# ykojima4020/mae_clip

Hardware: NVIDIA B200
Metric: contrastive loss fwd+bwd samples/s (higher is better)
Workload: dtype fp32 (fp16 hi+lo split operands, 3 tcgen05 passes, fp32 accumulate)

## Files before the change

mae_clip_b200/csrc/clip_loss_tc.cu:

```cuda
#include <stdlib.h>
#include <string.h>

#include "clip_loss.cuh"
#include "tc_ptx.cuh"

#include <type_traits>

namespace mc {
namespace tc {

using namespace ptx;


constexpr int kTileN = 128;
constexpr int kRowsCta = 64;
constexpr int kChunkBytes = 64 * 128;
constexpr int kThreads = 384;
constexpr int kEpiThreads = 256;
constexpr int kMaxSplit = 16;
constexpr int kIssuers = 1;

enum Phase { kStats = 0, kRowLoss = 1, kBwd = 2, kStatsZ = 3, kBwdW = 4, kBwdP = 5 };

constexpr int kOffA = 0;
// ... 1123 lines not shown
  __syncthreads();
  if (threadIdx.x < 32) {
    double t = (threadIdx.x < (blockDim.x >> 5)) ? sm[threadIdx.x] : 0.0;
    t = warp_sum(t);
    if (threadIdx.x == 0) *out = (float)t;
  }
}

__global__ void __launch_bounds__(1024) wscale_kernel(const float* __restrict__ r, const float* __restrict__ c,
                                                      const float* __restrict__ rz, const float* __restrict__ q, int B,
                                                      const float* __restrict__ scale,
                                                      const float* __restrict__ norm_i,
                                                      const float* __restrict__ norm_t, float inv_tau, float tau,
                                                      float* __restrict__ out) {
  __shared__ float sm[10][32];
  float v[10] = {-INFINITY, -INFINITY, 0.f, 0.f, 0.f, 0.f, -INFINITY, -INFINITY, -INFINITY, -INFINITY};
  auto take = [&](float ri, float ci, float zi, float qi, float ni, float nt) {
    v[0] = fmaxf(v[0], ri); v[1] = fmaxf(v[1], ci); v[2] = fmaxf(v[2], qi);
    v[4] = fmaxf(v[4], ni); v[5] = fmaxf(v[5], nt);
    v[6] = fmaxf(v[6], zi); v[7] = fmaxf(v[7], -ri); v[8] = fmaxf(v[8], -ci); v[9] = fmaxf(v[9], -zi);
  };
  int i0 = 0;
  const uintptr_t align = reinterpret_cast<uintptr_t>(r) | reinterpret_cast<uintptr_t>(c) | reinterpret_cast<uintptr_t>(rz) |
                          reinterpret_cast<uintptr_t>(q) | reinterpret_cast<uintptr_t>(norm_i) |
                          reinterpret_cast<uintptr_t>(norm_t);
  if ((align & 15) == 0) {
    const int B4 = B >> 2;
    for (int i = threadIdx.x; i < B4; i += blockDim.x) {
      const float4 a = reinterpret_cast<const float4*>(r)[i], b4 = reinterpret_cast<const float4*>(c)[i];
      const float4 z = reinterpret_cast<const float4*>(rz)[i], qq = reinterpret_cast<const float4*>(q)[i];
      const float4 ni = reinterpret_cast<const float4*>(norm_i)[i], nt = reinterpret_cast<const float4*>(norm_t)[i];
      take(a.x, b4.x, z.x, qq.x, ni.x, nt.x);
      take(a.y, b4.y, z.y, qq.y, ni.y, nt.y);
      take(a.z, b4.z, z.z, qq.z, ni.z, nt.z);
      take(a.w, b4.w, z.w, qq.w, ni.w, nt.w);
    }
    i0 = B4 << 2;
  }
  for (int i = i0 + threadIdx.x; i < B; i += blockDim.x) take(r[i], c[i], rz[i], q[i], norm_i[i], norm_t[i]);
  for (int k = 0; k < 10; ++k) {
    v[k] = warp_max(v[k]);
    if ((threadIdx.x & 31) == 0) sm[k][threadIdx.x >> 5] = v[k];
  }
  __syncthreads();
  if (threadIdx.x < 32) {
    for (int k = 0; k < 10; ++k) v[k] = warp_max(sm[k][threadIdx.x]);
    if (threadIdx.x == 0) {
      v[3] = scale[1];
      const float gmax = fmaxf(v[0] + v[1] + 2.f * v[4] * v[5] * inv_tau, 1.f);
      const float b1 = (2.f + v[2]) * v[3] * inv_tau;
      const float b3 = 2.f * gmax * v[3] * 0.5f * tau;
      const float bound = fmaxf(fmaxf(b1, b3), 1e-30f);
      int e;
      frexpf(bound, &e);
      int k = 15 - e;
      k = k < -60 ? -60 : (k > 60 ? 60 : k);
      out[0] = ldexpf(1.f, k);
      const float kL2e = 1.4426950408889634f;
      const float hi_rc = fmaxf(v[0], v[1]), lo_rc = -fmaxf(v[7], v[8]);
      const float hi_z = v[6], lo_z = -v[9];
      const bool fast = (hi_rc - lo_rc) * kL2e <= 60.f && (hi_z - lo_z) * kL2e <= 60.f;
      out[1] = fast ? 1.f : 0.f;
      out[2] = 0.5f * (hi_rc + lo_rc) * kL2e;
      out[3] = 0.5f * (hi_z + lo_z) * kL2e;
    }
  }
}

__global__ void __launch_bounds__(256) bwd_finalize_kernel(const float* __restrict__ part, int nsplit, int bpad,
                                                           int b, int D, float inv_2B,
                                                           const float* __restrict__ grad_loss,
                                                           const float* __restrict__ wscale,
                                                           float* __restrict__ dT, float* __restrict__ dI,
                                                           const int* __restrict__ gate = nullptr, int gate_want = 0) {
  if (gate != nullptr && *gate != gate_want) return;
  const float scale = (grad_loss ? *grad_loss : 1.f) * inv_2B / *wscale;
  const size_t n4 = (size_t)b * D / 4;
  const size_t plane = (size_t)bpad * D;
  for (size_t i = (size_t)blockIdx.x * blockDim.x + threadIdx.x; i < n4; i += (size_t)gridDim.x * blockDim.x) {
    float4 at = make_float4(0.f, 0.f, 0.f, 0.f), ai = at;
    for (int s = 0; s < nsplit; ++s) {
      const float4 a = reinterpret_cast<const float4*>(part + (size_t)s * 2 * plane)[i];
      const float4 c = reinterpret_cast<const float4*>(part + ((size_t)s * 2 + 1) * plane)[i];
      at.x += a.x; at.y += a.y; at.z += a.z; at.w += a.w;
      ai.x += c.x; ai.y += c.y; ai.z += c.z; ai.w += c.w;
    }
    reinterpret_cast<float4*>(dT)[i] = make_float4(at.x * scale, at.y * scale, at.z * scale, at.w * scale);
    reinterpret_cast<float4*>(dI)[i] = make_float4(ai.x * scale, ai.y * scale, ai.z * scale, ai.w * scale);
  }
}

constexpr int kCgThreads = 256;
constexpr int kCgStageA = 2 * 8192;
constexpr int kCgStages = 6;
constexpr int kCgMaxSplit = 8;
struct ColGradParams {
  int Bp, D;
  int w_rows;
  int row_offset;
  int j_first;
  int n_jblocks;
  int j_end;
  int ksplit, steps_per_split, steps;
  float* part;
  const int* gate;
};
__device__ __forceinline__ uint64_t smem_desc_mn_sw128(uint32_t saddr, uint32_t lbo_bytes) {
  uint64_t d = 0;
  d |= static_cast<uint64_t>((saddr & 0x3FFFFu) >> 4);
  d |= static_cast<uint64_t>(lbo_bytes >> 4) << 16;
  d |= static_cast<uint64_t>(1024 >> 4) << 32;
  d |= static_cast<uint64_t>(1) << 46;
  d |= static_cast<uint64_t>(2) << 61;
  return d;
}
__global__ void __launch_bounds__(kCgThreads, 1)
colgrad_kernel(const __grid_constant__ CUtensorMap map_w, const __grid_constant__ CUtensorMap map_t,
               const ColGradParams p) {
  if (p.gate != nullptr && *p.gate != 1) return;
  extern __shared__ uint8_t smem_raw[];
  const uint32_t raw = smem_u32(smem_raw);
  const uint32_t base = (raw + 1023u) & ~1023u;
  uint8_t* const sbase = smem_raw + (base - raw);
  const int D = p.D;
  const uint32_t b_bytes = (uint32_t)(D / 2) * 128u;
  const uint32_t stage_bytes = kCgStageA + b_bytes;
  const uint32_t bar0 = base + kCgStages * stage_bytes;
  auto bar = [&](int i) -> uint32_t { return bar0 + 8u * i; };
  enum { kFull = 0, kEmpty = kCgStages, kAccFull = 2 * kCgStages, kAccEmpty = 2 * kCgStages + 2, kBars = 2 * kCgStages + 4 };
  uint32_t* const tmem_slot = reinterpret_cast<uint32_t*>(sbase + kCgStages * stage_bytes + 8 * kBars);

  const int warp = __shfl_sync(0xffffffffu, (int)(threadIdx.x >> 5), 0), lane = threadIdx.x & 31;
  const uint32_t rank = cluster_ctarank();
  const bool leader = rank == 0;
  const int pair_id = blockIdx.x >> 1, npairs = gridDim.x >> 1;
  const int njobs = p.n_jblocks * p.ksplit;

  if (threadIdx.x == 0) {
    for (int s = 0; s < kCgStages; ++s) { mbar_init(bar(kFull + s), 1); mbar_init(bar(kEmpty + s), 1); }
    for (int i = 0; i < 2; ++i) { mbar_init(bar(kAccFull + i), 1); mbar_init(bar(kAccEmpty + i), 2 * 128); }
    fence_mbar_init();
    prefetch_tmap(&map_w);
    prefetch_tmap(&map_t);
  }
  if (warp == 1) {
    tmem_alloc_pair(smem_u32(tmem_slot), 512);
    tmem_relinquish_pair();
  }
  tc_fence_before();
  cluster_sync_all();
  tc_fence_after();
  const uint32_t tmem_base = *tmem_slot;

  if (warp == 0) {
    if (elect_one()) {
      uint32_t it = 0;
      for (int job = pair_id; job < njobs; job += npairs) {
        const int jb = job / p.ksplit, ks = job % p.ksplit;
        const int j0 = p.j_first + jb * 256 + (int)rank * 128;
        const int s0 = ks * p.steps_per_split, s1 = min(s0 + p.steps_per_split, p.steps);
        for (int st = s0; st < s1; ++st, ++it) {
          const uint32_t slot = it % kCgStages, par = (it / kCgStages) & 1;
          mbar_wait(bar(kEmpty + slot), par ^ 1);
          const uint32_t fb = bar(kFull + slot), sa = base + slot * stage_bytes;
          if (leader) mbar_arrive_expect_tx(fb, 2u * stage_bytes);
          const int i0 = st * 64;
          tma_load_2d_pair(sa, &map_w, fb, j0, i0);
          tma_load_2d_pair(sa + 8192, &map_w, fb, j0 + 64, i0);
          tma_load_2d_pair(sa + kCgStageA, &map_t, fb, p.row_offset + i0, D + (int)rank * (D / 2));
        }
      }
    }
  } else if (warp == 1) {
    if (leader && elect_one()) {
      const uint32_t idesc = idesc_f16(256, D) | (1u << 15);
      uint32_t it = 0, jj = 0;
      for (int job = pair_id; job < njobs; job += npairs) {
        const int ks = job % p.ksplit;
        const int s0 = ks * p.steps_per_split, s1 = min(s0 + p.steps_per_split, p.steps);
        if (s0 >= s1) continue;
        const uint32_t buf = jj & 1, use = jj >> 1;
        ++jj;
        mbar_wait(bar(kAccEmpty + buf), (use & 1) ^ 1);
        tc_fence_after();
        const uint32_t tacc = tmem_base + buf * (uint32_t)D;
        for (int st = s0; st < s1; ++st, ++it) {
          const uint32_t slot = it % kCgStages, par = (it / kCgStages) & 1;
          mbar_wait(bar(kFull + slot), par);
          tc_fence_after();
          const uint32_t sa = base + slot * stage_bytes;
          const uint64_t bd = smem_desc_sw128(sa + kCgStageA);
#pragma unroll
          for (int k4 = 0; k4 < 4; ++k4)
            mma_f16_pair(tacc, smem_desc_mn_sw128(sa + k4 * 2048, 8192), desc_advance_k(bd, k4), idesc,
                         (st > s0 || k4 > 0) ? 1u : 0u);
          mma_commit_pair(bar(kEmpty + slot), 3);
        }
        mma_commit_pair(bar(kAccFull + buf), 3);
      }
    }
  } else if (warp >= 4) {
    const int q = warp - 4;
    uint32_t jj = 0;
    for (int job = pair_id; job < njobs; job += npairs) {
      const int jb = job / p.ksplit, ks = job % p.ksplit;
      const int lrow = jb * 256 + (int)rank * 128 + q * 32 + lane;
      const bool ok = p.j_first + lrow < p.j_end;
      const int s0 = ks * p.steps_per_split;
      const bool empty = s0 >= p.steps;
      const uint32_t buf = jj & 1, use = jj >> 1;
      if (!empty) ++jj;
      float* out = p.part + ((size_t)ks * p.n_jblocks * 256 + lrow) * D;
      if (!empty) {
        mbar_wait(bar(kAccFull + buf), use & 1);
        tc_fence_after();
      }
      for (int c0 = 0; c0 < D; c0 += 32) {
        float v[32];
        if (!empty) {
          tmem_ld32(tmem_base + ((uint32_t)(q * 32) << 16) + buf * (uint32_t)D + c0, v);
          tmem_ld_wait();
        } else {
#pragma unroll
          for (int e = 0; e < 32; ++e) v[e] = 0.f;
        }
        if (ok) {
#pragma unroll
          for (int e = 0; e < 32; e += 4)
            *reinterpret_cast<float4*>(out + c0 + e) = make_float4(v[e], v[e + 1], v[e + 2], v[e + 3]);
        }
      }
      if (!empty) {
        tc_fence_before();
        mbar_arrive_cluster(bar(kAccEmpty + buf), 0);
      }
    }
  }
  tc_fence_before();
  cluster_sync_all();
  if (warp == 1) tmem_dealloc_pair(tmem_base, 512);
}

__global__ void __launch_bounds__(256) bwd_rows_finalize_kernel(const float* __restrict__ part, int nsplit, int bpad,
                                                                int b, int D, float inv_2B,
                                                                const float* __restrict__ grad_loss,
                                                                const float* __restrict__ wscale,
                                                                float* __restrict__ dT, float* __restrict__ dIz) {
  const float scale = (grad_loss ? *grad_loss : 1.f) * inv_2B / *wscale;
  const size_t n4 = (size_t)b * D / 4;
  const size_t plane = (size_t)bpad * D;
  for (size_t i = (size_t)blockIdx.x * blockDim.x + threadIdx.x; i < n4; i += (size_t)gridDim.x * blockDim.x) {
    float4 at = make_float4(0.f, 0.f, 0.f, 0.f), ai = at;
    for (int s = 0; s < nsplit; ++s) {
      const float4 a = reinterpret_cast<const float4*>(part + (size_t)s * 2 * plane)[i];
      const float4 c = reinterpret_cast<const float4*>(part + ((size_t)s * 2 + 1) * plane)[i];
      at.x += a.x; at.y += a.y; at.z += a.z; at.w += a.w;
      ai.x += c.x; ai.y += c.y; ai.z += c.z; ai.w += c.w;
    }
    reinterpret_cast<float4*>(dT)[i] = make_float4(at.x * scale, at.y * scale, at.z * scale, at.w * scale);
    reinterpret_cast<float4*>(dIz)[i] = ai;
  }
}
__global__ void __launch_bounds__(256) bwd_rows_split_finalize_kernel(const float* __restrict__ part_r, int nsplit_r,
                                                                      size_t plane_r, const float* __restrict__ part_p,
                                                                      size_t plane_p, int b, int D, float inv_2B,
                                                                      const float* __restrict__ grad_loss,
                                                                      const float* __restrict__ wscale,
                                                                      float* __restrict__ dT, float* __restrict__ dIz,
                                                                      const int* __restrict__ gate) {
  if (gate != nullptr && *gate != 1) return;
  const float scale = (grad_loss ? *grad_loss : 1.f) * inv_2B / *wscale;
  const size_t n4 = (size_t)b * D / 4;
  for (size_t i = (size_t)blockIdx.x * blockDim.x + threadIdx.x; i < n4; i += (size_t)gridDim.x * blockDim.x) {
    float4 at = reinterpret_cast<const float4*>(part_p)[i];
    for (int s = 0; s < nsplit_r; ++s) {
      const float4 a = reinterpret_cast<const float4*>(part_r + (size_t)s * plane_r)[i];
      at.x += a.x; at.y += a.y; at.z += a.z; at.w += a.w;
    }
    reinterpret_cast<float4*>(dT)[i] = make_float4(at.x * scale, at.y * scale, at.z * scale, at.w * scale);
    reinterpret_cast<float4*>(dIz)[i] = reinterpret_cast<const float4*>(part_p + plane_p)[i];
  }
}
__global__ void __launch_bounds__(256) bwd_cols_finalize_kernel(const float* __restrict__ part, int ksplit, size_t plane,
                                                                int rows, int D, float inv_2B,
                                                                const float* __restrict__ grad_loss,
                                                                const float* __restrict__ wscale,
                                                                const float* __restrict__ dIz, float* __restrict__ dI,
                                                                const int* __restrict__ gate) {
  if (gate != nullptr && *gate != 1) return;
  const float scale = (grad_loss ? *grad_loss : 1.f) * inv_2B / *wscale;
  const size_t n4 = (size_t)rows * D / 4;
  for (size_t i = (size_t)blockIdx.x * blockDim.x + threadIdx.x; i < n4; i += (size_t)gridDim.x * blockDim.x) {
    float4 a = dIz ? reinterpret_cast<const float4*>(dIz)[i] : make_float4(0.f, 0.f, 0.f, 0.f);
    for (int s = 0; s < ksplit; ++s) {
      const float4 c = reinterpret_cast<const float4*>(part + (size_t)s * plane)[i];
      a.x += c.x; a.y += c.y; a.z += c.z; a.w += c.w;
    }
    reinterpret_cast<float4*>(dI)[i] = make_float4(a.x * scale, a.y * scale, a.z * scale, a.w * scale);
  }
}

constexpr int kRgThreads = 384;
constexpr int kRgRowsCta = 128;
constexpr int kRgSlotBytes = 32768;
constexpr int kRgSlots = 3;
constexpr int kRgOffA = 0;
constexpr int kRgOffRing = 65536;
constexpr int kRgOffW = kRgOffRing + kRgSlots * kRgSlotBytes;
constexpr int kRgOffXT = kRgOffW + 2 * 16384;
constexpr int kRgOffConst = kRgOffXT + 2 * 16384;
constexpr int kRgOffBar = kRgOffConst + 2048;
constexpr int kRgSmemBytes = kRgOffBar + 256 + 512;
enum RgBar {
  kRgFull0 = 0, kRgEmpty0 = 3, kRgAFull = 6, kRgJobDone = 7, kRgTmemFull0 = 8, kRgTmemEmpty0 = 10, kRgWFull0 = 12,
  kRgXTFull0 = 14, kRgGradDone0 = 16, kRgAccFull = 18, kRgAccEmpty = 19, kRgCstFull0 = 20, kRgCstEmpty0 = 22, kRgNumBars = 24
};
struct RowGradParams {
  int b, B, Bp, D, row_offset;
  int n_row_blocks, n_tiles, nsplit, tiles_per_split, bpad;
  float inv_tau;
  const float* scale;
  const float *r, *c, *q;
  const float* wscale;
  float* part;
  __half* wout;
  const int* gate;
};
template <int PASSES>
__global__ void __launch_bounds__(kRgThreads, 1)
rowgrad_kernel(const __grid_constant__ CUtensorMap map_a_hi, const __grid_constant__ CUtensorMap map_a_lo,
               const __grid_constant__ CUtensorMap map_b_hi, const __grid_constant__ CUtensorMap map_b_lo,
               const __grid_constant__ CUtensorMap map_t, const RowGradParams p) {
  if (p.gate != nullptr && *p.gate != 1) return;
  extern __shared__ __align__(1024) uint8_t smem_raw[];
  const uint32_t raw = smem_u32(smem_raw);
  const uint32_t base = (raw + 1023u) & ~1023u;
  if (base - raw > 512u) __trap();
  uint8_t* const sbase = smem_raw + (base - raw);
  const uint32_t bar0 = base + kRgOffBar;
  auto bar = [&](int i) -> uint32_t { return bar0 + 8u * i; };
  uint32_t* const tmem_slot = reinterpret_cast<uint32_t*>(sbase + kRgOffBar + 8 * kRgNumBars);

  const int warp = __shfl_sync(0xffffffffu, (int)(threadIdx.x >> 5), 0), lane = threadIdx.x & 31;
  const uint32_t rank = cluster_ctarank();
  const bool leader = rank == 0;
  const int pair_id = blockIdx.x >> 1, npairs = gridDim.x >> 1;
  const int D = p.D, nkc = D >> 6;
  const int njobs = p.n_row_blocks * p.nsplit;
  const uint32_t xt_bytes = (uint32_t)(D / 2) * 128u;

  if (threadIdx.x == 0) {
    for (int s = 0; s < kRgSlots; ++s) { mbar_init(bar(kRgFull0 + s), 1); mbar_init(bar(kRgEmpty0 + s), 1); }
    mbar_init(bar(kRgAFull), 1);
    mbar_init(bar(kRgJobDone), 1);
    for (int i = 0; i < 2; ++i) {
      mbar_init(bar(kRgTmemFull0 + i), 1);
      mbar_init(bar(kRgTmemEmpty0 + i), 2 * 256);
      mbar_init(bar(kRgWFull0 + i), 2 * 128);
      mbar_init(bar(kRgXTFull0 + i), 1);
      mbar_init(bar(kRgGradDone0 + i), 1);
      mbar_init(bar(kRgCstFull0 + i), 32);
      mbar_init(bar(kRgCstEmpty0 + i), 256);
    }
    mbar_init(bar(kRgAccFull), 1);
    mbar_init(bar(kRgAccEmpty), 2 * 256);
    fence_mbar_init();
    prefetch_tmap(&map_a_hi); prefetch_tmap(&map_a_lo); prefetch_tmap(&map_b_hi); prefetch_tmap(&map_b_lo);
    prefetch_tmap(&map_t);
  }
  if (warp == 1) {
    tmem_alloc_pair(smem_u32(tmem_slot), 512);
    tmem_relinquish_pair();
  }
  tc_fence_before();
  cluster_sync_all();
  tc_fence_after();
  const uint32_t tmem_base = *tmem_slot;
  constexpr uint32_t kAcc = 256;

  if (warp == 0) {
    if (elect_one()) {
      uint32_t it = 0, jj = 0;
      for (int job = pair_id; job < njobs; job += npairs, ++jj) {
        const int rb = job / p.nsplit, sp = job % p.nsplit;
        const int row_a = p.row_offset + rb * 256 + (int)rank * kRgRowsCta;
        const int t0 = sp * p.tiles_per_split, t1 = min(t0 + p.tiles_per_split, p.n_tiles);
        mbar_wait(bar(kRgJobDone), (jj & 1) ^ 1);
        if (leader) mbar_arrive_expect_tx(bar(kRgAFull), 2u * (uint32_t)nkc * 16384u);
        for (int c = 0; c < nkc; ++c) tma_load_2d_pair(base + kRgOffA + c * 16384, &map_a_hi, bar(kRgAFull), D + c * 64, row_a);
        for (int t = t0; t < t1; ++t) {
          const int j0 = t * kTileN + 64 * (int)rank;
          for (int c = 0; c < nkc; ++c, ++it) {
            const uint32_t slot = it % kRgSlots, par = (it / kRgSlots) & 1;
            mbar_wait(bar(kRgEmpty0 + slot), par ^ 1);
            const uint32_t fb = bar(kRgFull0 + slot), sb = base + kRgOffRing + slot * kRgSlotBytes;
            if (leader) mbar_arrive_expect_tx(fb, PASSES == 3 ? 2u * kRgSlotBytes : 2u * 8192u);
            if (PASSES == 3) tma_load_2d_pair(sb, &map_a_lo, fb, D + c * 64, row_a);
            tma_load_2d_pair(sb + 16384, &map_b_hi, fb, c * 64, j0);
            if (PASSES == 3) tma_load_2d_pair(sb + 24576, &map_b_lo, fb, c * 64, j0);
          }
        }
      }
    }
  } else if (warp == 2) {
    if (elect_one()) {
      uint32_t tt = 0;
      for (int job = pair_id; job < njobs; job += npairs) {
        const int sp = job % p.nsplit;
        const int t0 = sp * p.tiles_per_split, t1 = min(t0 + p.tiles_per_split, p.n_tiles);
        for (int t = t0; t < t1; ++t, ++tt) {
          for (int h = 0; h < 2; ++h) {
            mbar_wait(bar(kRgGradDone0 + h), (tt & 1) ^ 1);
            const uint32_t fb = bar(kRgXTFull0 + h);
            if (leader) mbar_arrive_expect_tx(fb, 2u * xt_bytes);
            tma_load_2d_pair(base + kRgOffXT + h * 16384, &map_t, fb, t * kTileN + 64 * h, (int)rank * (D / 2));
          }
        }
      }
    }
  } else if (warp == 3) {
    float* const consts = reinterpret_cast<float*>(sbase + kRgOffConst);
    const float kL2e = 1.4426950408889634f;
    const bool fast = p.wscale[1] != 0.f;
    const float m_rc = p.wscale[2];
    uint32_t tt = 0;
    for (int job = pair_id; job < njobs; job += npairs) {
      const int sp = job % p.nsplit;
      const int t0 = sp * p.tiles_per_split, t1 = min(t0 + p.tiles_per_split, p.n_tiles);
      for (int t = t0; t < t1; ++t, ++tt) {
        float vc[4], vq[4];
#pragma unroll
        for (int u = 0; u < 4; ++u) {
          const int jcol = t * kTileN + lane + 32 * u;
          const bool ok = jcol < p.B;
          vc[u] = ok ? p.c[jcol] : 0.f;
          vq[u] = ok ? p.q[jcol] : 0.f;
        }
        mbar_wait(bar(kRgCstEmpty0 + (tt & 1)), ((tt >> 1) & 1) ^ 1);
        float* dst = consts + (tt & 1) * 256;
#pragma unroll
        for (int u = 0; u < 4; ++u) {
          const int col = lane + 32 * u;
          const bool ok = t * kTileN + col < p.B;
          const float c2 = vc[u] * kL2e;
          if (fast) {
            dst[col] = ok ? ex2f(m_rc - c2) * vq[u] : 0.f;
          } else {
            dst[col] = -c2;
            dst[128 + col] = vq[u];
          }
        }
        mbar_arrive_local(bar(kRgCstFull0 + (tt & 1)));
      }
    }
  } else if (warp == 1) {
    if (leader && elect_one()) {
      constexpr uint32_t idesc_s = idesc_f16(256, kTileN);
      const uint32_t idesc_g = idesc_f16(256, D);
      const uint32_t tDT = tmem_base + kAcc;
      uint32_t it = 0, tt = 0, gt = 0, jj = 0;
      auto grad_tile = [&](bool first_of_job) {
        for (int h = 0; h < 2; ++h) {
          mbar_wait(bar(kRgWFull0 + h), gt & 1);
          mbar_wait(bar(kRgXTFull0 + h), gt & 1);
          tc_fence_after();
          const uint64_t wd = smem_desc_sw128(base + kRgOffW + h * 16384), xd = smem_desc_sw128(base + kRgOffXT + h * 16384);
#pragma unroll
          for (int ks = 0; ks < 4; ++ks)
            mma_f16_pair(tDT, desc_advance_k(wd, ks), desc_advance_k(xd, ks), idesc_g, (first_of_job && h == 0 && ks == 0) ? 0u : 1u);
          mma_commit_pair(bar(kRgGradDone0 + h), 3);
        }
        ++gt;
      };
      for (int job = pair_id; job < njobs; job += npairs, ++jj) {
        const int sp = job % p.nsplit;
        const int t0 = sp * p.tiles_per_split, t1 = min(t0 + p.tiles_per_split, p.n_tiles);
        mbar_wait(bar(kRgAFull), jj & 1);
        tc_fence_after();
        for (int t = t0; t < t1; ++t, ++tt) {
          const uint32_t buf = tt & 1, use = tt >> 1;
          mbar_wait(bar(kRgTmemEmpty0 + buf), (use & 1) ^ 1);
          tc_fence_after();
          const uint32_t tS = tmem_base + buf * 128;
          for (int c = 0; c < nkc; ++c, ++it) {
            const uint32_t slot = it % kRgSlots, par = (it / kRgSlots) & 1;
            mbar_wait(bar(kRgFull0 + slot), par);
            tc_fence_after();
            const uint32_t sb = base + kRgOffRing + slot * kRgSlotBytes;
            const uint64_t aT = smem_desc_sw128(base + kRgOffA + c * 16384), aTl = smem_desc_sw128(sb);
            const uint64_t bI = smem_desc_sw128(sb + 16384), bIl = smem_desc_sw128(sb + 24576);
#pragma unroll
            for (int ks = 0; ks < 4; ++ks) {
              const uint64_t kT = desc_advance_k(aT, ks), kb = desc_advance_k(bI, ks);
              mma_f16_pair(tS, kT, kb, idesc_s, (c > 0 || ks > 0) ? 1u : 0u);
              if (PASSES == 3) {
                mma_f16_pair(tS, kT, desc_advance_k(bIl, ks), idesc_s, 1u);
                mma_f16_pair(tS, desc_advance_k(aTl, ks), kb, idesc_s, 1u);
              }
            }
            mma_commit_pair(bar(kRgEmpty0 + slot), 3);
          }
          mma_commit_pair(bar(kRgTmemFull0 + buf), 3);
          if (t == t0) {
            mbar_wait(bar(kRgAccEmpty), (jj & 1) ^ 1);
            tc_fence_after();
          } else {
            grad_tile(t - 1 == t0);
          }
        }
        grad_tile(t1 - 1 == t0);
        mma_commit_pair(bar(kRgAccFull), 3);
        mma_commit_pair(bar(kRgJobDone), 3);
      }
    }
    __syncwarp();
  } else if (warp >= 4) {
    const int q4 = warp & 3, h = (warp - 4) >> 2;
    const int m = q4 * 32 + lane;
    const uint32_t lane_field = (uint32_t)(q4 * 32) << 16;
    const float* const consts = reinterpret_cast<const float*>(sbase + kRgOffConst);
    const float kL2e = 1.4426950408889634f;
    const float inv_s = p.scale[1], inv_s2 = p.scale[2];
    const float cS2 = inv_s2 * p.inv_tau * kL2e;
    const float wS = inv_s * p.inv_tau * p.wscale[0];
    const bool fast = p.wscale[1] != 0.f;
    const float m_rc = p.wscale[2];
    uint32_t tt = 0, jj = 0;
    for (int job = pair_id; job < njobs; job += npairs, ++jj) {
      const int rb = job / p.nsplit, sp = job % p.nsplit;
      const int t0 = sp * p.tiles_per_split, t1 = min(t0 + p.tiles_per_split, p.n_tiles);
      const int lrow = rb * 256 + (int)rank * kRgRowsCta + m;
      const int gi = p.row_offset + lrow;
      const bool row_ok = lrow < p.b;
      const float r2_i = row_ok ? p.r[gi] * kL2e : 0.f;
      const float fC_i = ex2f(r2_i - m_rc);
      const float wrow = row_ok ? wS : 0.f;
      for (int t = t0; t < t1; ++t, ++tt) {
        const uint32_t buf = tt & 1, use = tt >> 1;
        mbar_wait(bar(kRgCstFull0 + (tt & 1)), (tt >> 1) & 1);
        const float* cst = consts + (tt & 1) * 256 + 64 * h;
        mbar_wait(bar(kRgTmemFull0 + buf), use & 1);
        tc_fence_after();
        const uint32_t tS = tmem_base + buf * 128 + lane_field + 64 * h;
        uint32_t wp[32];
#pragma unroll
        for (int half = 0; half < 2; ++half) {
          float v[32];
          tmem_ld32(tS + 32 * half, v);
          tmem_ld_wait();
          if (half == 1) {
            tc_fence_before();
            mbar_arrive_cluster(bar(kRgTmemEmpty0 + buf), 0);
          }
#pragma unroll
          for (int e = 0; e < 32; e += 4) {
            const float4 f0 = *reinterpret_cast<const float4*>(cst + 32 * half + e);
            const float4 f1 = fast ? make_float4(0.f, 0.f, 0.f, 0.f) : *reinterpret_cast<const float4*>(cst + 128 + 32 * half + e);
            const float k0[4] = {f0.x, f0.y, f0.z, f0.w}, k1[4] = {f1.x, f1.y, f1.z, f1.w};
            float w[4];
#pragma unroll
            for (int u = 0; u < 4; ++u) {
              const float a = v[e + u];
              const float e1 = ex2f(fmaf(a, cS2, -r2_i));
              float dS;
              if (fast) dS = e1 * fmaf(fC_i, k0[u], 1.f);
              else dS = fmaf(ex2f(fmaf(a, cS2, k0[u])), k1[u], e1);
              w[u] = dS * wrow;
            }
            __half2 x = __floats2half2_rn(w[0], w[1]), y = __floats2half2_rn(w[2], w[3]);
            wp[16 * half + (e >> 1)] = *reinterpret_cast<uint32_t*>(&x);
            wp[16 * half + (e >> 1) + 1] = *reinterpret_cast<uint32_t*>(&y);
          }
        }
        mbar_wait(bar(kRgGradDone0 + h), (tt & 1) ^ 1);
        uint8_t* wsm = sbase + kRgOffW + h * 16384 + m * 128;
#pragma unroll
        for (int k = 0; k < 8; ++k)
          *reinterpret_cast<uint4*>(wsm + ((k ^ (m & 7)) * 16)) = make_uint4(wp[4 * k], wp[4 * k + 1], wp[4 * k + 2], wp[4 * k + 3]);
        fence_proxy_async_smem();
        mbar_arrive_cluster(bar(kRgWFull0 + h), 0);
        uint4* wg = reinterpret_cast<uint4*>(p.wout + (size_t)lrow * p.Bp + (size_t)t * kTileN + 64 * h);
#pragma unroll
        for (int k = 0; k < 8; ++k) wg[k] = make_uint4(wp[4 * k], wp[4 * k + 1], wp[4 * k + 2], wp[4 * k + 3]);
        mbar_arrive_local(bar(kRgCstEmpty0 + (tt & 1)));
      }
      mbar_wait(bar(kRgAccFull), jj & 1);
      tc_fence_after();
      float* out = p.part + ((size_t)sp * p.bpad + lrow) * D + h * (D / 2);
      for (int c0 = 0; c0 < D / 2; c0 += 32) {
        float v[32];
        tmem_ld32(tmem_base + lane_field + kAcc + h * (D / 2) + c0, v);
        tmem_ld_wait();
#pragma unroll
        for (int e = 0; e < 32; e += 4) *reinterpret_cast<float4*>(out + c0 + e) = make_float4(v[e], v[e + 1], v[e + 2], v[e + 3]);
      }
      tc_fence_before();
      mbar_arrive_cluster(bar(kRgAccEmpty), 0);
    }
  }
  tc_fence_before();
  cluster_sync_all();
  if (warp == 1) tmem_dealloc_pair(tmem_base, 512);
}

enum RsKind { kRsS = 0, kRsZ = 1 };
constexpr int kRsThreads = 384;
constexpr int kRsNBuf = 4;
constexpr int kRsOffScratch = 212992;
constexpr int kRsOffBar = kRsOffScratch + 2048;
constexpr int kRsSmemBytes = kRsOffBar + 256 + 512;
enum RsBar { kRsFull0 = 0, kRsEmpty0 = 5, kRsAFull = 10, kRsJobDone = 11, kRsTmemFull0 = 12, kRsTmemEmpty0 = 16, kRsNumBars = 20 };
struct RowSweepParams {
  int b, B, Bp, D, row_offset;
  int n_row_blocks, n_tiles, nsplit, tiles_per_split, bpad;
  int chunk_k, chunk_blocks, chunk_m;
  int tri;
  float inv_tau, half_tau;
  const float* scale;
  float2* part;
  float* colpart;
  uint8_t* flags_out;
  const float *norm_i, *norm_t;
  const float* tile_min_zjj2;
  int pk;
  const float* rho;
  const float* tile_max_rho;
  const float* tile_max_n;
  const int* gate;
  int gate_want;
};
__device__ __forceinline__ int rs_njobs(const RowSweepParams& p) {
  if (p.chunk_k < 0) return p.n_row_blocks * p.nsplit;
  return p.chunk_blocks * (p.chunk_k + 1) * p.chunk_m + p.chunk_k * p.chunk_blocks * p.chunk_m;
}
__device__ __forceinline__ void rs_job(const RowSweepParams& p, int job, int& rb, int& sp) {
  if (p.chunk_k < 0) { rb = job / p.nsplit; sp = job % p.nsplit; return; }
  const int w = (p.chunk_k + 1) * p.chunk_m, first = p.chunk_blocks * w;
  if (job < first) { rb = p.chunk_k * p.chunk_blocks + job / w; sp = job % w; return; }
  job -= first;
  rb = job / p.chunk_m;
  sp = p.chunk_k * p.chunk_m + job % p.chunk_m;
}
template <int KIND>
__device__ __forceinline__ void rs_tiles(const RowSweepParams& p, int rb, int sp, int& t0, int& t1) {
  t0 = sp * p.tiles_per_split;
  t1 = min(t0 + p.tiles_per_split, p.n_tiles);
  if (KIND == kRsZ && p.tri) t0 = max(t0, 2 * rb);
}
template <int KIND, int PASSES>
__global__ void __launch_bounds__(kRsThreads, 1)
rowsweep_kernel(const __grid_constant__ CUtensorMap map_a_hi, const __grid_constant__ CUtensorMap map_a_lo,
                const __grid_constant__ CUtensorMap map_b_hi, const __grid_constant__ CUtensorMap map_b_lo,
                const RowSweepParams p) {
  constexpr int kSlotBytes_ = KIND == kRsS ? 32768 : 16384;
  constexpr int kSlots = KIND == kRsS ? 4 : 5;
  constexpr int kOffRing = KIND == kRsS ? 65536 : 131072;
  static_assert(kOffRing + kSlots * kSlotBytes_ <= kRsOffScratch, "ring overlaps the scratch");
  extern __shared__ __align__(1024) uint8_t smem_raw[];
  const uint32_t raw = smem_u32(smem_raw);
  const uint32_t base = (raw + 1023u) & ~1023u;
  if (base - raw > 512u) __trap();
  uint8_t* const sbase = smem_raw + (base - raw);
  const uint32_t bar0 = base + kRsOffBar;
  auto bar = [&](int i) -> uint32_t { return bar0 + 8u * i; };
  uint32_t* const tmem_slot = reinterpret_cast<uint32_t*>(sbase + kRsOffBar + 8 * kRsNumBars);

  const int warp = __shfl_sync(0xffffffffu, (int)(threadIdx.x >> 5), 0), lane = threadIdx.x & 31;
  const uint32_t rank = cluster_ctarank();
  const bool leader = rank == 0;
  const int pair_id = blockIdx.x >> 1, npairs = gridDim.x >> 1;
  if (KIND == kRsZ && p.gate != nullptr && *p.gate != p.gate_want) return;
  const int D = p.D, nkc = D >> 6;
  const int nkz = KIND == kRsS ? nkc : p.pk;
  const int njobs = rs_njobs(p);
  const int n_res = KIND == kRsS ? nkc : 2 * nkz;

  if (threadIdx.x == 0) {
    for (int s = 0; s < kSlots; ++s) { mbar_init(bar(kRsFull0 + s), 1); mbar_init(bar(kRsEmpty0 + s), 1); }
    mbar_init(bar(kRsAFull), 1);
    mbar_init(bar(kRsJobDone), 1);
    for (int i = 0; i < kRsNBuf; ++i) { mbar_init(bar(kRsTmemFull0 + i), 1); mbar_init(bar(kRsTmemEmpty0 + i), 2 * 256); }
    fence_mbar_init();
    prefetch_tmap(&map_a_hi); prefetch_tmap(&map_a_lo); prefetch_tmap(&map_b_hi); prefetch_tmap(&map_b_lo);
  }
  if (warp == 1) {
    tmem_alloc_pair(smem_u32(tmem_slot), 512);
    tmem_relinquish_pair();
  }
  tc_fence_before();
  cluster_sync_all();
  tc_fence_after();
  const uint32_t tmem_base = *tmem_slot;

  if (warp == 0) {
    if (elect_one()) {
      uint32_t it = 0, jj = 0;
      for (int job = pair_id; job < njobs; job += npairs) {
        int rb, sp, t0, t1;
        rs_job(p, job, rb, sp);
        rs_tiles<KIND>(p, rb, sp, t0, t1);
        if (t0 >= t1) continue;
        const int row_a = p.row_offset + rb * 256 + (int)rank * 128;
        mbar_wait(bar(kRsJobDone), (jj & 1) ^ 1);
        ++jj;
        if (leader) mbar_arrive_expect_tx(bar(kRsAFull), 2u * (uint32_t)n_res * 16384u);
        if (KIND == kRsS) {
          for (int c = 0; c < nkc; ++c) tma_load_2d_pair(base + c * 16384, &map_a_hi, bar(kRsAFull), D + c * 64, row_a);
        } else {
          for (int c = 0; c < nkz; ++c) {
            tma_load_2d_pair(base + c * 16384, &map_a_hi, bar(kRsAFull), c * 64, row_a);
            tma_load_2d_pair(base + (nkc + c) * 16384, &map_a_hi, bar(kRsAFull), D + c * 64, row_a);
          }
        }
        for (int t = t0; t < t1; ++t) {
          const int j0 = t * kTileN + 64 * (int)rank;
          for (int c = 0; c < nkz; ++c, ++it) {
            const uint32_t slot = it % kSlots, par = (it / kSlots) & 1;
            mbar_wait(bar(kRsEmpty0 + slot), par ^ 1);
            const uint32_t fb = bar(kRsFull0 + slot), sb = base + kOffRing + slot * kSlotBytes_;
            if (leader) mbar_arrive_expect_tx(fb, (KIND == kRsS && PASSES != 3) ? 2u * 8192u : 2u * kSlotBytes_);
            if (KIND == kRsS) {
              if (PASSES == 3) tma_load_2d_pair(sb, &map_a_lo, fb, D + c * 64, row_a);
              tma_load_2d_pair(sb + 16384, &map_b_hi, fb, c * 64, j0);
              if (PASSES == 3) tma_load_2d_pair(sb + 24576, &map_b_lo, fb, c * 64, j0);
            } else {
              tma_load_2d_pair(sb, &map_b_hi, fb, c * 64, j0);
              tma_load_2d_pair(sb + 8192, &map_b_hi, fb, D + c * 64, j0);
            }
          }
        }
      }
    }
  } else if (warp == 1) {
    if (leader && elect_one()) {
      constexpr uint32_t idesc = idesc_f16(256, kTileN);
      uint32_t it = 0, tt = 0, jj = 0;
      for (int job = pair_id; job < njobs; job += npairs) {
        int rb, sp, t0, t1;
        rs_job(p, job, rb, sp);
        rs_tiles<KIND>(p, rb, sp, t0, t1);
        if (t0 >= t1) continue;
        mbar_wait(bar(kRsAFull), jj & 1);
        ++jj;
        tc_fence_after();
        for (int t = t0; t < t1; ++t, ++tt) {
          const uint32_t buf = tt % kRsNBuf, use = tt / kRsNBuf;
          mbar_wait(bar(kRsTmemEmpty0 + buf), (use & 1) ^ 1);
          tc_fence_after();
          const uint32_t tD = tmem_base + buf * 128;
          for (int c = 0; c < nkz; ++c, ++it) {
            const uint32_t slot = it % kSlots, par = (it / kSlots) & 1;
            mbar_wait(bar(kRsFull0 + slot), par);
            tc_fence_after();
            const uint32_t sb = base + kOffRing + slot * kSlotBytes_;
            if (KIND == kRsS) {
              const uint64_t aT = smem_desc_sw128(base + c * 16384), aTl = smem_desc_sw128(sb);
              const uint64_t bI = smem_desc_sw128(sb + 16384), bIl = smem_desc_sw128(sb + 24576);
#pragma unroll
              for (int ks = 0; ks < 4; ++ks) {
                const uint64_t kT = desc_advance_k(aT, ks), kb = desc_advance_k(bI, ks);
                mma_f16_pair(tD, kT, kb, idesc, (c > 0 || ks > 0) ? 1u : 0u);
                if (PASSES == 3) {
                  mma_f16_pair(tD, kT, desc_advance_k(bIl, ks), idesc, 1u);
                  mma_f16_pair(tD, desc_advance_k(aTl, ks), kb, idesc, 1u);
                }
              }
            } else {
              const uint64_t aI = smem_desc_sw128(base + c * 16384), aT = smem_desc_sw128(base + (nkc + c) * 16384);
              const uint64_t bI = smem_desc_sw128(sb), bT = smem_desc_sw128(sb + 8192);
#pragma unroll
              for (int ks = 0; ks < 4; ++ks) {
                mma_f16_pair(tD, desc_advance_k(aI, ks), desc_advance_k(bI, ks), idesc, (c > 0 || ks > 0) ? 1u : 0u);
                mma_f16_pair(tD, desc_advance_k(aT, ks), desc_advance_k(bT, ks), idesc, 1u);
              }
            }
            mma_commit_pair(bar(kRsEmpty0 + slot), 3);
          }
          mma_commit_pair(bar(kRsTmemFull0 + buf), 3);
        }
        mma_commit_pair(bar(kRsJobDone), 3);
      }
    }
    __syncwarp();
  } else if (warp >= 4) {
    const int q4 = warp & 3, h = (warp - 4) >> 2;
    const int m = q4 * 32 + lane;
    const uint32_t lane_field = (uint32_t)(q4 * 32) << 16;
    float* const scratch = reinterpret_cast<float*>(sbase + kRsOffScratch);
    const float kL2e = 1.4426950408889634f;
    const float inv_s2 = p.scale[2];
    const float cS2 = inv_s2 * p.inv_tau * kL2e, cZ2 = inv_s2 * p.half_tau * kL2e;
    const float zmargin2 = kProbeMargin2 + (1.f / 512.f) * (8.f * (float)D * inv_s2 * p.half_tau * kL2e);
    uint32_t tt = 0;
    for (int job = pair_id; job < njobs; job += npairs) {
      int rb, sp, t0, t1;
      rs_job(p, job, rb, sp);
      const int lrow = rb * 256 + (int)rank * 128 + m;
      const int gi = p.row_offset + lrow;
      const bool row_ok = lrow < p.b;
      rs_tiles<KIND>(p, rb, sp, t0, t1);
      if (t0 >= t1) continue;
      float mS = -INFINITY, sS = 0.f;
      float zii2 = 0.f, rho2 = 0.f, rnd2 = 0.f;
      if (KIND == kRsZ && row_ok) {
        const float ni = p.norm_i[gi], nt = p.norm_t[gi];
        zii2 = (ni * ni + nt * nt) * p.half_tau * kL2e;
        if (p.rho != nullptr) {
          rho2 = p.rho[gi] * p.half_tau * kL2e * 1.0001f;
          rnd2 = sqrtf(ni * ni + nt * nt) * p.half_tau * kL2e * (1.07f / 1024.f);
        }
      }
      const int rb128 = rb * 2 + (int)rank;
      for (int t = t0; t < t1; ++t, ++tt) {
        const uint32_t buf = tt % kRsNBuf, use = tt / kRsNBuf;
        mbar_wait(bar(kRsTmemFull0 + buf), use & 1);
        tc_fence_after();
        const uint32_t tD = tmem_base + buf * 128 + lane_field + 64 * h;
        const bool ragged = (t + 1) * kTileN > p.B;
        float cmz = -INFINITY;
#pragma unroll
        for (int half = 0; half < 2; ++half) {
          float v[32];
          tmem_ld32(tD + 32 * half, v);
          tmem_ld_wait();
          if (half == 1) {
            tc_fence_before();
            mbar_arrive_cluster(bar(kRsTmemEmpty0 + buf), 0);
          }
          const int jl0 = 64 * h + 32 * half;
          if (ragged) {
            const int jlim = p.B - t * kTileN;
#pragma unroll
            for (int e = 0; e < 32; ++e) if (jl0 + e >= jlim) v[e] = -INFINITY;
          }
          float c4[4] = {fmaxf(v[0], v[4]), fmaxf(v[1], v[5]), fmaxf(v[2], v[6]), fmaxf(v[3], v[7])};
#pragma unroll
          for (int e = 8; e < 32; e += 4) {
#pragma unroll
            for (int u = 0; u < 4; ++u) c4[u] = fmaxf(c4[u], v[e + u]);
          }
          const float cm = fmaxf(fmaxf(c4[0], c4[1]), fmaxf(c4[2], c4[3]));
          if (KIND == kRsZ) {
            cmz = fmaxf(cmz, cm);
          } else {
            float a[32];
            if (cm != -INFINITY) {
              float a4[4] = {0.f, 0.f, 0.f, 0.f};
#pragma unroll
              for (int e = 0; e < 32; e += 4) {
#pragma unroll
                for (int u = 0; u < 4; ++u) { a[e + u] = ex2f((v[e + u] - cm) * cS2); a4[u] += a[e + u]; }
              }
              const float mn = fmaxf(mS, cm);
              sS = sS * ex2f((mS - mn) * cS2) + ((a4[0] + a4[1]) + (a4[2] + a4[3])) * ex2f((cm - mn) * cS2);
              mS = mn;
            } else {
#pragma unroll
              for (int e = 0; e < 32; ++e) a[e] = 0.f;
            }
            const int g32 = (rb * 256 + (int)rank * 128 + q4 * 32) >> 5;
            float* const cp_out = p.colpart + (size_t)g32 * p.Bp + (size_t)t * kTileN + jl0 + lane;
            bool col_done = false;
            if (!ragged && __all_sync(0xffffffffu, row_ok)) {
              float M;
              asm volatile("redux.sync.max.f32 %0, %1, 0xffffffff;" : "=f"(M) : "f"(cm));
              const float w = ex2f((cm - M) * cS2);
#pragma unroll
              for (int e = 0; e < 32; ++e) a[e] *= w;
#pragma unroll
              for (int s2 = 16; s2 >= 1; s2 >>= 1) {
                const bool up = (lane & s2) != 0;
#pragma unroll
                for (int k = 0; k < s2; ++k) {
                  const float keep = up ? a[k + s2] : a[k], send = up ? a[k] : a[k + s2];
                  a[k] = keep + __shfl_xor_sync(0xffffffffu, send, s2);
                }
              }
              if (__all_sync(0xffffffffu, a[0] >= 7.8886e-31f)) {
                *cp_out = fmaf(M, cS2, lg2f(a[0]));
                col_done = true;
              }
            }
            if (!col_done) {
              float* cmx = scratch + (warp - 4) * 32;
              __syncwarp();
#pragma unroll
              for (int e = 0; e < 32; ++e) {
                float cme;
                const float in = row_ok ? v[e] : -INFINITY;
                asm volatile("redux.sync.max.f32 %0, %1, 0xffffffff;" : "=f"(cme) : "f"(in));
                if (lane == 0) cmx[e] = cme;
                const float ref = cme == -INFINITY ? 0.f : cme;
                a[e] = row_ok ? ex2f((v[e] - ref) * cS2) : 0.f;
              }
              __syncwarp();
              const float cm_own = cmx[lane];
#pragma unroll
              for (int s2 = 16; s2 >= 1; s2 >>= 1) {
                const bool up = (lane & s2) != 0;
#pragma unroll
                for (int k = 0; k < s2; ++k) {
                  const float keep = up ? a[k + s2] : a[k], send = up ? a[k] : a[k + s2];
                  a[k] = keep + __shfl_xor_sync(0xffffffffu, send, s2);
                }
              }
              *cp_out = cm_own == -INFINITY ? -INFINITY : fmaf(cm_own, cS2, lg2f(a[0]));
            }
          }
        }
        if (KIND == kRsZ) {
          float z2 = -INFINITY, zm2 = zmargin2;
          if (row_ok) {
            z2 = cmz * cZ2;
            if (p.rho != nullptr) {
              z2 += fmaf(rho2, p.tile_max_rho[t], rnd2 * p.tile_max_n[t]);
              zm2 = kProbeMargin2 + 8.f * (float)D * 2.98e-8f * cZ2;
            }
          }
          const bool hit = z2 >= zii2 - kFlagTheta2 - zm2;
          if (__any_sync(0xffffffffu, hit) && lane == 0) p.flags_out[(size_t)rb128 * p.n_tiles + t] = 1;
          if (p.tri && t != rb128) {
            const float wm = warp_max(z2);
            if (lane == 0 && wm >= p.tile_min_zjj2[t] - kFlagTheta2 - zm2) p.flags_out[(size_t)t * p.n_tiles + rb128] = 1;
          }
        }
      }
      if (KIND == kRsS) {
        named_bar_sync(2, 256);
        float* sc = scratch + 256;
        if (h == 1) { sc[m] = mS * cS2; sc[128 + m] = sS; }
        named_bar_sync(2, 256);
        if (h == 0) {
          OnlineLse2 l;
          l.m = mS * cS2; l.s = sS;
          l.merge(sc[m], sc[128 + m]);
          p.part[(size_t)sp * p.bpad + lrow] = make_float2(l.m, l.s);
        }
      }
    }
  }
  tc_fence_before();
  cluster_sync_all();
  if (warp == 1) tmem_dealloc_pair(tmem_base, 512);
}

__global__ void __launch_bounds__(128) tile_min_zjj_kernel(const float* __restrict__ norm_i, const float* __restrict__ norm_t,
                                                           const float* __restrict__ rho, int B, float half_tau,
                                                           float* __restrict__ out, float* __restrict__ out_rho,
                                                           float* __restrict__ out_n) {
  __shared__ float sm[4], sr[4], sn[4];
  const int j = blockIdx.x * 128 + threadIdx.x;
  float z = INFINITY, r = 0.f, n = 0.f;
  if (j < B) {
    const float ni = norm_i[j], nt = norm_t[j];
    z = (ni * ni + nt * nt) * half_tau * 1.4426950408889634f;
    r = rho[j];
    n = sqrtf(ni * ni + nt * nt);
  }
  for (int o = 16; o > 0; o >>= 1) {
    z = fminf(z, __shfl_xor_sync(0xffffffffu, z, o));
    r = fmaxf(r, __shfl_xor_sync(0xffffffffu, r, o));
    n = fmaxf(n, __shfl_xor_sync(0xffffffffu, n, o));
  }
  if ((threadIdx.x & 31) == 0) { sm[threadIdx.x >> 5] = z; sr[threadIdx.x >> 5] = r; sn[threadIdx.x >> 5] = n; }
  __syncthreads();
  if (threadIdx.x == 0) {
    out[blockIdx.x] = fminf(fminf(sm[0], sm[1]), fminf(sm[2], sm[3]));
    out_rho[blockIdx.x] = fmaxf(fmaxf(sr[0], sr[1]), fmaxf(sr[2], sr[3]));
    out_n[blockIdx.x] = fmaxf(fmaxf(sn[0], sn[1]), fmaxf(sn[2], sn[3]));
  }
}
__global__ void __launch_bounds__(256) probe_hopeless_kernel(const float* __restrict__ tile_min_zjj2,
                                                             const float* __restrict__ tile_max_rho, int n_valid,
                                                             float half_tau, int* __restrict__ hopeless) {
  __shared__ int cnt;
  if (threadIdx.x == 0) cnt = 0;
  __syncthreads();
  int c = 0;
  for (int t = threadIdx.x; t < n_valid; t += blockDim.x) {
    const float r = tile_max_rho[t];
    c += r * r * half_tau * 1.4426950408889634f >= tile_min_zjj2[t] - kFlagTheta2 - kProbeMargin2;
  }
  for (int o = 16; o > 0; o >>= 1) c += __shfl_xor_sync(0xffffffffu, c, o);
  if ((threadIdx.x & 31) == 0 && c) atomicAdd(&cnt, c);
  __syncthreads();
  if (threadIdx.x == 0 && 2 * cnt > n_valid) *hopeless = 1;
}
__global__ void __launch_bounds__(1024) probe_gate_kernel(uint8_t* __restrict__ flags, int n, int limit, int* __restrict__ gate) {
  __shared__ int cnt;
  if (threadIdx.x == 0) cnt = 0;
  __syncthreads();
  int c = 0;
  const bool vec = (reinterpret_cast<uintptr_t>(flags) & 15) == 0 && n % 16 == 0;
  if (vec) {
    for (int i = threadIdx.x; i < n / 16; i += blockDim.x) {
      const uint4 w = reinterpret_cast<const uint4*>(flags)[i];
      c += __popc(w.x) + __popc(w.y) + __popc(w.z) + __popc(w.w);
    }
  } else {
    for (int i = threadIdx.x; i < n; i += blockDim.x) c += flags[i] != 0;
  }
  for (int o = 16; o > 0; o >>= 1) c += __shfl_xor_sync(0xffffffffu, c, o);
  if ((threadIdx.x & 31) == 0 && c) atomicAdd(&cnt, c);
  __syncthreads();
  const bool redo = cnt > limit || gate[1] != 0;
  if (redo) {
    if (vec) for (int i = threadIdx.x; i < n / 16; i += blockDim.x) reinterpret_cast<uint4*>(flags)[i] = make_uint4(0u, 0u, 0u, 0u);
    else for (int i = threadIdx.x; i < n; i += blockDim.x) flags[i] = 0;
  }
  if (threadIdx.x == 0) *gate = redo ? 1 : 0;
}
__global__ void __launch_bounds__(256) rowsweep_finalize_kernel(const float2* __restrict__ part, int nsplit, int bpad, int b,
                                                                float* __restrict__ r) {
  const int i = blockIdx.x * blockDim.x + threadIdx.x;
  if (i >= b) return;
  OnlineLse2 l;
  l.init();
  for (int s = 0; s < nsplit; ++s) {
    const float2 v = part[(size_t)s * bpad + i];
    l.merge(v.x, v.y);
  }
  r[i] = (l.m + log2f(l.s)) * kLn2;
}

typedef CUresult (*EncodeTiledFn)(CUtensorMap*, CUtensorMapDataType, cuuint32_t, void*, const cuuint64_t*,
                                  const cuuint64_t*, const cuuint32_t*, const cuuint32_t*, CUtensorMapInterleave,
                                  CUtensorMapSwizzle, CUtensorMapL2promotion, CUtensorMapFloatOOBfill);

static EncodeTiledFn encode_fn() {
  static EncodeTiledFn fn = nullptr;
  if (!fn) {
    void* f = nullptr;
    cudaDriverEntryPointQueryResult q;
    if (cudaGetDriverEntryPoint("cuTensorMapEncodeTiled", &f, cudaEnableDefault, &q) == cudaSuccess &&
        q == cudaDriverEntryPointSuccess)
      fn = reinterpret_cast<EncodeTiledFn>(f);
  }
  return fn;
}

static int make_map(CUtensorMap* m, const void* ptr, uint64_t rows, uint64_t cols, uint32_t box_rows) {
  EncodeTiledFn fn = encode_fn();
  MC_REQUIRE(fn != nullptr, MC_ERR_CUDA, "cuTensorMapEncodeTiled is not available from the driver");
  cuuint64_t dims[2] = {cols, rows};
  cuuint64_t strides[1] = {cols * sizeof(__half)};
  cuuint32_t box[2] = {64, box_rows};
  cuuint32_t estr[2] = {1, 1};
  CUresult r = fn(m, CU_TENSOR_MAP_DATA_TYPE_FLOAT16, 2, const_cast<void*>(ptr), dims, strides, box, estr,
                  CU_TENSOR_MAP_INTERLEAVE_NONE, CU_TENSOR_MAP_SWIZZLE_128B, CU_TENSOR_MAP_L2_PROMOTION_L2_256B,
                  CU_TENSOR_MAP_FLOAT_OOB_FILL_NONE);
  MC_REQUIRE(r == CUDA_SUCCESS, MC_ERR_CUDA, "cuTensorMapEncodeTiled failed (%d)", (int)r);
  return MC_OK;
}

struct Split {
  int n_row_blocks, n_tiles, nsplit, tiles_per_split, bpad;
};
constexpr double kOvhStats = 1.5, kOvhRowLoss = 0.5, kOvhBwd = 6.0;
template <int PHASE> constexpr double phase_ovh() { return (PHASE == kBwd || PHASE == kBwdW || PHASE == kBwdP) ? kOvhBwd : (PHASE == kRowLoss ? kOvhRowLoss : kOvhStats); }
static Split choose_split(int b, int B, double ovh = kOvhRowLoss, int align = 1) {
// ... 987 lines not shown
```

Baseline: 8.692 million.

## Keep A-lo operand resident in smem instead of reloading it per tile

```diff
diff --git a/mae_clip_b200/csrc/clip_loss_tc.cu b/mae_clip_b200/csrc/clip_loss_tc.cu
--- a/mae_clip_b200/csrc/clip_loss_tc.cu
+++ b/mae_clip_b200/csrc/clip_loss_tc.cu
@@ -1449,18 +1449,17 @@
 
 constexpr int kRgThreads = 384;
 constexpr int kRgRowsCta = 128;
-constexpr int kRgSlotBytes = 32768;
-constexpr int kRgSlots = 3;
+constexpr int kRgRingBytes = 98304;
 constexpr int kRgOffA = 0;
 constexpr int kRgOffRing = 65536;
-constexpr int kRgOffW = kRgOffRing + kRgSlots * kRgSlotBytes;
+constexpr int kRgOffW = kRgOffRing + kRgRingBytes;
 constexpr int kRgOffXT = kRgOffW + 2 * 16384;
 constexpr int kRgOffConst = kRgOffXT + 2 * 16384;
 constexpr int kRgOffBar = kRgOffConst + 2048;
 constexpr int kRgSmemBytes = kRgOffBar + 256 + 512;
 enum RgBar {
-  kRgFull0 = 0, kRgEmpty0 = 3, kRgAFull = 6, kRgJobDone = 7, kRgTmemFull0 = 8, kRgTmemEmpty0 = 10, kRgWFull0 = 12,
-  kRgXTFull0 = 14, kRgGradDone0 = 16, kRgAccFull = 18, kRgAccEmpty = 19, kRgCstFull0 = 20, kRgCstEmpty0 = 22, kRgNumBars = 24
+  kRgFull0 = 0, kRgEmpty0 = 4, kRgAFull = 8, kRgJobDone = 9, kRgTmemFull0 = 10, kRgTmemEmpty0 = 12, kRgWFull0 = 14,
+  kRgXTFull0 = 16, kRgGradDone0 = 18, kRgAccFull = 20, kRgAccEmpty = 21, kRgCstFull0 = 22, kRgCstEmpty0 = 24, kRgNumBars = 26
 };
 struct RowGradParams {
   int b, B, Bp, D, row_offset;
@@ -1479,6 +1478,11 @@
                const __grid_constant__ CUtensorMap map_b_hi, const __grid_constant__ CUtensorMap map_b_lo,
                const __grid_constant__ CUtensorMap map_t, const RowGradParams p) {
   if (p.gate != nullptr && *p.gate != 1) return;
+  constexpr bool kResLo = PASSES == 3;
+  constexpr int kSlots = kResLo ? 2 : 4;
+  constexpr uint32_t kSlotB = kResLo ? 16384 : 8192;
+  constexpr uint32_t kRing = kResLo ? kRgOffRing + 65536 : kRgOffRing;
+  static_assert(kRing + kSlots * kSlotB <= (uint32_t)kRgOffW, "ring overflows its region");
   extern __shared__ __align__(1024) uint8_t smem_raw[];
   const uint32_t raw = smem_u32(smem_raw);
   const uint32_t base = (raw + 1023u) & ~1023u;
@@ -1497,7 +1501,7 @@
   const uint32_t xt_bytes = (uint32_t)(D / 2) * 128u;
 
   if (threadIdx.x == 0) {
-    for (int s = 0; s < kRgSlots; ++s) { mbar_init(bar(kRgFull0 + s), 1); mbar_init(bar(kRgEmpty0 + s), 1); }
+    for (int s = 0; s < kSlots; ++s) { mbar_init(bar(kRgFull0 + s), 1); mbar_init(bar(kRgEmpty0 + s), 1); }
     mbar_init(bar(kRgAFull), 1);
     mbar_init(bar(kRgJobDone), 1);
     for (int i = 0; i < 2; ++i) {
@@ -1533,18 +1537,20 @@
         const int row_a = p.row_offset + rb * 256 + (int)rank * kRgRowsCta;
         const int t0 = sp * p.tiles_per_split, t1 = min(t0 + p.tiles_per_split, p.n_tiles);
         mbar_wait(bar(kRgJobDone), (jj & 1) ^ 1);
-        if (leader) mbar_arrive_expect_tx(bar(kRgAFull), 2u * (uint32_t)nkc * 16384u);
-        for (int c = 0; c < nkc; ++c) tma_load_2d_pair(base + kRgOffA + c * 16384, &map_a_hi, bar(kRgAFull), D + c * 64, row_a);
+        if (leader) mbar_arrive_expect_tx(bar(kRgAFull), (kResLo ? 4u : 2u) * (uint32_t)nkc * 16384u);
+        for (int c = 0; c < nkc; ++c) {
+          tma_load_2d_pair(base + kRgOffA + c * 16384, &map_a_hi, bar(kRgAFull), D + c * 64, row_a);
+          if (kResLo) tma_load_2d_pair(base + kRgOffRing + c * 16384, &map_a_lo, bar(kRgAFull), D + c * 64, row_a);
+        }
         for (int t = t0; t < t1; ++t) {
           const int j0 = t * kTileN + 64 * (int)rank;
           for (int c = 0; c < nkc; ++c, ++it) {
-            const uint32_t slot = it % kRgSlots, par = (it / kRgSlots) & 1;
+            const uint32_t slot = it % kSlots, par = (it / kSlots) & 1;
             mbar_wait(bar(kRgEmpty0 + slot), par ^ 1);
-            const uint32_t fb = bar(kRgFull0 + slot), sb = base + kRgOffRing + slot * kRgSlotBytes;
-            if (leader) mbar_arrive_expect_tx(fb, PASSES == 3 ? 2u * kRgSlotBytes : 2u * 8192u);
-            if (PASSES == 3) tma_load_2d_pair(sb, &map_a_lo, fb, D + c * 64, row_a);
-            tma_load_2d_pair(sb + 16384, &map_b_hi, fb, c * 64, j0);
-            if (PASSES == 3) tma_load_2d_pair(sb + 24576, &map_b_lo, fb, c * 64, j0);
+            const uint32_t fb = bar(kRgFull0 + slot), sb = base + kRing + slot * kSlotB;
+            if (leader) mbar_arrive_expect_tx(fb, 2u * kSlotB);
+            tma_load_2d_pair(sb, &map_b_hi, fb, c * 64, j0);
+            if (kResLo) tma_load_2d_pair(sb + 8192, &map_b_lo, fb, c * 64, j0);
           }
         }
       }
@@ -1630,12 +1636,13 @@
           tc_fence_after();
           const uint32_t tS = tmem_base + buf * 128;
           for (int c = 0; c < nkc; ++c, ++it) {
-            const uint32_t slot = it % kRgSlots, par = (it / kRgSlots) & 1;
+            const uint32_t slot = it % kSlots, par = (it / kSlots) & 1;
             mbar_wait(bar(kRgFull0 + slot), par);
             tc_fence_after();
-            const uint32_t sb = base + kRgOffRing + slot * kRgSlotBytes;
-            const uint64_t aT = smem_desc_sw128(base + kRgOffA + c * 16384), aTl = smem_desc_sw128(sb);
-            const uint64_t bI = smem_desc_sw128(sb + 16384), bIl = smem_desc_sw128(sb + 24576);
+            const uint32_t sb = base + kRing + slot * kSlotB;
+            const uint64_t aT = smem_desc_sw128(base + kRgOffA + c * 16384);
+            const uint64_t aTl = smem_desc_sw128(base + kRgOffRing + c * 16384);
+            const uint64_t bI = smem_desc_sw128(sb), bIl = smem_desc_sw128(sb + 8192);
 #pragma unroll
             for (int ks = 0; ks < 4; ++ks) {
               const uint64_t kT = desc_advance_k(aT, ks), kb = desc_advance_k(bI, ks);
@@ -1799,9 +1806,10 @@
 rowsweep_kernel(const __grid_constant__ CUtensorMap map_a_hi, const __grid_constant__ CUtensorMap map_a_lo,
                 const __grid_constant__ CUtensorMap map_b_hi, const __grid_constant__ CUtensorMap map_b_lo,
                 const RowSweepParams p) {
-  constexpr int kSlotBytes_ = KIND == kRsS ? 32768 : 16384;
-  constexpr int kSlots = KIND == kRsS ? 4 : 5;
-  constexpr int kOffRing = KIND == kRsS ? 65536 : 131072;
+  constexpr bool kOneRes = KIND == kRsS && PASSES != 3;
+  constexpr int kSlotBytes_ = kOneRes ? 32768 : 16384;
+  constexpr int kSlots = kOneRes ? 4 : 5;
+  constexpr int kOffRing = kOneRes ? 65536 : 131072;
   static_assert(kOffRing + kSlots * kSlotBytes_ <= kRsOffScratch, "ring overlaps the scratch");
   extern __shared__ __align__(1024) uint8_t smem_raw[];
   const uint32_t raw = smem_u32(smem_raw);
@@ -1820,7 +1828,7 @@
   const int D = p.D, nkc = D >> 6;
   const int nkz = KIND == kRsS ? nkc : p.pk;
   const int njobs = rs_njobs(p);
-  const int n_res = KIND == kRsS ? nkc : 2 * nkz;
+  const int n_res = kOneRes ? nkc : (KIND == kRsS ? 2 * nkc : 2 * nkz);
 
   if (threadIdx.x == 0) {
     for (int s = 0; s < kSlots; ++s) { mbar_init(bar(kRsFull0 + s), 1); mbar_init(bar(kRsEmpty0 + s), 1); }
@@ -1852,7 +1860,10 @@
         ++jj;
         if (leader) mbar_arrive_expect_tx(bar(kRsAFull), 2u * (uint32_t)n_res * 16384u);
         if (KIND == kRsS) {
-          for (int c = 0; c < nkc; ++c) tma_load_2d_pair(base + c * 16384, &map_a_hi, bar(kRsAFull), D + c * 64, row_a);
+          for (int c = 0; c < nkc; ++c) {
+            tma_load_2d_pair(base + c * 16384, &map_a_hi, bar(kRsAFull), D + c * 64, row_a);
+            if (PASSES == 3) tma_load_2d_pair(base + 65536 + c * 16384, &map_a_lo, bar(kRsAFull), D + c * 64, row_a);
+          }
         } else {
           for (int c = 0; c < nkz; ++c) {
             tma_load_2d_pair(base + c * 16384, &map_a_hi, bar(kRsAFull), c * 64, row_a);
@@ -1867,9 +1878,8 @@
             const uint32_t fb = bar(kRsFull0 + slot), sb = base + kOffRing + slot * kSlotBytes_;
             if (leader) mbar_arrive_expect_tx(fb, (KIND == kRsS && PASSES != 3) ? 2u * 8192u : 2u * kSlotBytes_);
             if (KIND == kRsS) {
-              if (PASSES == 3) tma_load_2d_pair(sb, &map_a_lo, fb, D + c * 64, row_a);
-              tma_load_2d_pair(sb + 16384, &map_b_hi, fb, c * 64, j0);
-              if (PASSES == 3) tma_load_2d_pair(sb + 24576, &map_b_lo, fb, c * 64, j0);
+              tma_load_2d_pair(sb + (PASSES == 3 ? 0 : 16384), &map_b_hi, fb, c * 64, j0);
+              if (PASSES == 3) tma_load_2d_pair(sb + 8192, &map_b_lo, fb, c * 64, j0);
             } else {
               tma_load_2d_pair(sb, &map_b_hi, fb, c * 64, j0);
               tma_load_2d_pair(sb + 8192, &map_b_hi, fb, D + c * 64, j0);
@@ -1901,8 +1911,8 @@
             tc_fence_after();
             const uint32_t sb = base + kOffRing + slot * kSlotBytes_;
             if (KIND == kRsS) {
-              const uint64_t aT = smem_desc_sw128(base + c * 16384), aTl = smem_desc_sw128(sb);
-              const uint64_t bI = smem_desc_sw128(sb + 16384), bIl = smem_desc_sw128(sb + 24576);
+              const uint64_t aT = smem_desc_sw128(base + c * 16384), aTl = smem_desc_sw128(base + 65536 + c * 16384);
+              const uint64_t bI = smem_desc_sw128(sb + (PASSES == 3 ? 0 : 16384)), bIl = smem_desc_sw128(sb + 8192);
 #pragma unroll
               for (int ks = 0; ks < 4; ++ks) {
                 const uint64_t kT = desc_advance_k(aT, ks), kb = desc_advance_k(bI, ks);
```

Measured after the change: 8.805 million, median of 6. About the same (+1.3%).
